# davidbau/rewriting

Hardware: NVIDIA H100
Metric: StyleGAN2-256 images/sec (higher is better)
Workload: dtype bf16x3 (3-term split bf16 operands, fp32 accumulate; fp32 in/out)

## Files before the change

rewriting_b200/csrc/conv_tc.cu:

```cuda
#include <cstdlib>
#include <cstring>

#include "rw_common.cuh"
#include "rw_kernels.h"

namespace rw {

namespace {

constexpr int BM = 128;
constexpr int BN = 128;
constexpr int BK = 64;
constexpr int MMA_K = 16;
constexpr int kStages = 3;
constexpr int kNumThreads = 288;
constexpr int kTmaWarp = 8;
constexpr int kChunkKB = 8;

struct ConvSmem {
  static constexpr int kABytes = BM * BK * 2;
  static constexpr int kBBytes = BN * BK * 2;
  static constexpr int kStageBytes = 2 * kABytes + 2 * kBBytes;
  static constexpr int kTotal = kStages * kStageBytes + 1024  + 256 ;
};

struct Barriers {
  uint64_t full[kStages];
  uint64_t empty[kStages];
};

__device__ __forceinline__ void decode_tile(int tile, int nphase, int nsched, int& ph, int& mn) {
  mn = tile / nphase;
  ph = tile - mn * nphase;
  if (nphase > 1) ph = (ph + ((nsched % nphase) == 0 ? tile / nsched : mn)) % nphase;
}

template <int EPI>
__global__ void __launch_bounds__(kNumThreads, 1)
conv_tc_kernel(const __grid_constant__ CUtensorMap map_a_hi,
               const __grid_constant__ CUtensorMap map_a_lo,
               const __grid_constant__ CUtensorMap map_w_hi,
               const __grid_constant__ CUtensorMap map_w_lo, const ConvTcParams p) {
  extern __shared__ uint8_t smem_raw[];
  uint8_t* smem = reinterpret_cast<uint8_t*>((reinterpret_cast<uintptr_t>(smem_raw) + 1023) &
                                             ~static_cast<uintptr_t>(1023));
  using S = ConvSmem;
  Barriers* bars = reinterpret_cast<Barriers*>(smem + kStages * S::kStageBytes);

  const int warp = threadIdx.x >> 5;
  const int lane = threadIdx.x & 31;
  const int nsched = gridDim.x;

  const int m_tiles = (p.rows + BM - 1) / BM;
  const int n_tiles = p.Cout / BN;
  const int mn_tiles = m_tiles * n_tiles;
  const int num_tiles = mn_tiles * p.nphase;
  const int kb_per_tap = p.Cin / BK;

  if (warp == kTmaWarp && lane == 0) {
    tma_prefetch_desc(&map_a_hi);
    tma_prefetch_desc(&map_a_lo);
    tma_prefetch_desc(&map_w_hi);
    tma_prefetch_desc(&map_w_lo);
    for (int s = 0; s < kStages; ++s) {
      mbar_init(&bars->full[s], 1);
      mbar_init(&bars->empty[s], 2);
    }
    fence_mbar_init();
  }
  __syncthreads();

  if (warp == kTmaWarp) {
    if (lane == 0) {
      int stage = 0;
      uint32_t phase = 0;
      for (int tile = blockIdx.x; tile < num_tiles; tile += nsched) {
        int ph, mn;
        decode_tile(tile, p.nphase, nsched, ph, mn);
        const int n0 = (mn % n_tiles) * BN;
        const int m0 = (mn / n_tiles) * BM;
        for (int t = 0; t < p.ph_ntaps[ph]; ++t) {
          const int arow = m0 + p.ph_shift[ph][t];
          const int wcol = p.ph_kofs[ph][t];
          const int acol = p.ph_acol[ph][t];
          for (int kb = 0; kb < kb_per_tap; ++kb) {
            mbar_wait(&bars->empty[stage], phase ^ 1u);
            uint8_t* st = smem + stage * S::kStageBytes;
            mbar_expect_tx(&bars->full[stage], S::kStageBytes);
            tma_load_2d(st, &map_a_hi, &bars->full[stage], acol + kb * BK, arow);
            tma_load_2d(st + S::kABytes, &map_a_lo, &bars->full[stage], acol + kb * BK, arow);
            tma_load_2d(st + 2 * S::kABytes, &map_w_hi, &bars->full[stage], wcol + kb * BK, n0);
            tma_load_2d(st + 2 * S::kABytes + S::kBBytes, &map_w_lo, &bars->full[stage],
                        wcol + kb * BK, n0);
            if (++stage == kStages) { stage = 0; phase ^= 1u; }
          }
        }
      }
    }
    return;
  }

  const int wg = threadIdx.x >> 7;
  const int g = lane >> 2, c = lane & 3;
  const int img = p.Hp * p.Wp;
  int stage = 0;
  uint32_t phase = 0;
  for (int tile = blockIdx.x; tile < num_tiles; tile += nsched) {
    int ph, mn;
    decode_tile(tile, p.nphase, nsched, ph, mn);
    const int num_kb = p.ph_ntaps[ph] * kb_per_tap;
    const int n_tile = mn % n_tiles;
    const int n0 = n_tile * BN;
    const int m0 = (mn / n_tiles) * BM;

    float acc[64], d[64];
#pragma unroll
    for (int j = 0; j < 64; ++j) acc[j] = 0.f;
    for (int kb0 = 0; kb0 < num_kb; kb0 += kChunkKB) {
      const int kb_end = (kb0 + kChunkKB < num_kb) ? kb0 + kChunkKB : num_kb;
      for (int kb = kb0; kb < kb_end; ++kb) {
        mbar_wait(&bars->full[stage], phase);
        const uint32_t sa = smem_u32(smem + stage * S::kStageBytes);
        const uint64_t da_hi = make_smem_desc(sa + wg * (S::kABytes / 2), 16, 1024);
        const uint64_t da_lo = make_smem_desc(sa + S::kABytes + wg * (S::kABytes / 2), 16, 1024);
        const uint64_t db_hi = make_smem_desc(sa + 2 * S::kABytes, 16, 1024);
        const uint64_t db_lo = make_smem_desc(sa + 2 * S::kABytes + S::kBBytes, 16, 1024);
        wgmma_fence();
#pragma unroll
        for (int kk = 0; kk < BK / MMA_K; ++kk) {
          const uint64_t adv = static_cast<uint64_t>((kk * MMA_K * 2) >> 4);
          wgmma_m64n128<0, 0>(d, da_lo + adv, db_hi + adv, ((kb - kb0) | kk) != 0);
          wgmma_m64n128<0, 0>(d, da_hi + adv, db_lo + adv, 1u);
          wgmma_m64n128<0, 0>(d, da_hi + adv, db_hi + adv, 1u);
        }
        wgmma_commit();
        wgmma_wait<0>();
        if ((threadIdx.x & 127) == 0) mbar_arrive(&bars->empty[stage]);
        if (++stage == kStages) { stage = 0; phase ^= 1u; }
      }
#pragma unroll
      for (int j = 0; j < 64; ++j) acc[j] += d[j];
    }

#pragma unroll
    for (int i = 0; i < 2; ++i) {
      const int prow = m0 + wg * 64 + (warp & 3) * 16 + g + 8 * i;
      const int b = prow / img;
      const int rem = prow - b * img;
      const int yy = rem / p.Wp;
      const int xx = rem - yy * p.Wp;
      const int Hv = p.ph_Hv[ph], Wv = p.ph_Wv[ph];
      const bool in_rows = prow < p.rows;
      const bool valid = in_rows && (yy < Hv) && (xx < Wv);
      const float* scl = (p.scale_bo && in_rows) ? p.scale_bo + static_cast<size_t>(b) * p.Cout : nullptr;
      float* outp = (p.out != nullptr && p.out_mode == 0 && valid)
                        ? p.out + p.ph_out_ofs[ph] + static_cast<size_t>(b) * p.out_sb +
                              static_cast<size_t>(yy) * p.out_sy + static_cast<size_t>(xx) * p.out_sx
                        : nullptr;
      if (EPI == 1 || !valid) {
        if (scl && (EPI == 1 || p.out_mode == 1)) {
#pragma unroll
          for (int j = 0; j < 16; ++j) {
            const float2 sv = __ldg(reinterpret_cast<const float2*>(scl + n0 + 8 * j + 2 * c));
            acc[4 * j + 2 * i] *= sv.x;
            acc[4 * j + 2 * i + 1] *= sv.y;
          }
        }
        if (EPI == 1 && outp) {
#pragma unroll
          for (int j = 0; j < 16; ++j)
#pragma unroll
            for (int e = 0; e < 2; ++e)
              outp[static_cast<size_t>(n0 + 8 * j + 2 * c + e) * p.out_sc] = acc[4 * j + 2 * i + e];
        }
      } else {
        float nz = 0.f;
        if (p.noise != nullptr)
          nz = __ldg(p.noise_w) * __ldg(p.noise + static_cast<size_t>(b) * p.noise_bstride +
                                        static_cast<size_t>(yy) * Wv + xx);
        const float act_gain = p.act_gain != 0.f ? p.act_gain : 1.4142135623730951f;
#pragma unroll
        for (int j = 0; j < 16; ++j)
#pragma unroll
          for (int e = 0; e < 2; ++e) {
            const int o = n0 + 8 * j + 2 * c + e;
            float t = acc[4 * j + 2 * i + e];
            if (scl) t *= __ldg(scl + o);
            t += nz;
            if (p.bias) t += __ldg(p.bias + o);
            if (p.act) t = (t > 0.f ? t : 0.2f * t) * act_gain;
            acc[4 * j + 2 * i + e] = t;
            if (outp) outp[static_cast<size_t>(o) * p.out_sc] = t;
          }
      }
      if (EPI == 0 && p.rgb_w != nullptr) {
        const float* rw0 = p.rgb_w + (static_cast<size_t>(valid ? b : 0) * 3) * p.Cout;
#pragma unroll
        for (int half = 0; half < 2; ++half) {
          float r0 = 0.f, r1 = 0.f, r2 = 0.f;
          if (valid) {
#pragma unroll
            for (int j = 8 * half; j < 8 * half + 8; ++j)
#pragma unroll
              for (int e = 0; e < 2; ++e) {
                const int o = n0 + 8 * j + 2 * c + e;
                const float t = acc[4 * j + 2 * i + e];
                r0 = fmaf(__ldg(rw0 + o), t, r0);
                r1 = fmaf(__ldg(rw0 + p.Cout + o), t, r1);
                r2 = fmaf(__ldg(rw0 + 2 * p.Cout + o), t, r2);
              }
          }
#pragma unroll
          for (int s = 1; s < 4; s <<= 1) {
            r0 += __shfl_xor_sync(0xffffffffu, r0, s);
            r1 += __shfl_xor_sync(0xffffffffu, r1, s);
            r2 += __shfl_xor_sync(0xffffffffu, r2, s);
          }
          if (valid && c == 0) {
            const size_t hw = static_cast<size_t>(Hv) * Wv;
            float* rp = p.rgb_part + ((static_cast<size_t>(n_tile * 2 + half) * p.B + b) * 3) * hw +
                        static_cast<size_t>(yy) * Wv + xx;
            rp[0] = r0;
            rp[hw] = r1;
            rp[2 * hw] = r2;
          }
        }
      }
      if (p.out != nullptr && p.out_mode == 1 && in_rows) {
        float* orow = p.out + (static_cast<size_t>(ph) * p.rows + prow) * p.Cout + n0 + 2 * c;
#pragma unroll
        for (int j = 0; j < 16; ++j)
          *reinterpret_cast<float2*>(orow + 8 * j) = make_float2(acc[4 * j + 2 * i], acc[4 * j + 2 * i + 1]);
      }
      if (EPI == 0 && p.next_hi != nullptr && in_rows) {
        const float* ns = p.next_scale + static_cast<size_t>(valid ? b : 0) * p.Cout + n0 + 2 * c;
        const size_t ofs = static_cast<size_t>(prow) * p.Cout + n0 + 2 * c;
        uint32_t* nh = reinterpret_cast<uint32_t*>(static_cast<__nv_bfloat16*>(p.next_hi) + ofs);
        uint32_t* nl = reinterpret_cast<uint32_t*>(static_cast<__nv_bfloat16*>(p.next_lo) + ofs);
#pragma unroll
        for (int j = 0; j < 16; ++j) {
          float k0 = 0.f, k1 = 0.f;
          if (valid) {
            const float2 sv = __ldg(reinterpret_cast<const float2*>(ns + 8 * j));
            k0 = sv.x * acc[4 * j + 2 * i];
            k1 = sv.y * acc[4 * j + 2 * i + 1];
          }
          const __nv_bfloat162 hh = __floats2bfloat162_rn(k0, k1);
          const float2 hf = __bfloat1622float2(hh);
          const __nv_bfloat162 ll = __floats2bfloat162_rn(k0 - hf.x, k1 - hf.y);
          nh[4 * j] = *reinterpret_cast<const uint32_t*>(&hh);
          nl[4 * j] = *reinterpret_cast<const uint32_t*>(&ll);
        }
      }
    }
  }
}

}

template <int EPI>
static int conv_tc_launch_epi(const ConvTcParams& p, const void* a_hi, const void* a_lo,
                              const void* w_hi, const void* w_lo, int wk_total,
                              cudaStream_t stream) {
  CUtensorMap ma_hi, ma_lo, mw_hi, mw_lo;
  int rc;
  const int a_cols = p.a_cols > 0 ? p.a_cols : p.Cin;
  if ((rc = make_tmap_2d_bf16(&ma_hi, a_hi, a_cols, p.rows, (uint64_t)a_cols * 2, BK, BM))) return rc;
  if ((rc = make_tmap_2d_bf16(&ma_lo, a_lo, a_cols, p.rows, (uint64_t)a_cols * 2, BK, BM))) return rc;
  if ((rc = make_tmap_2d_bf16(&mw_hi, w_hi, wk_total, p.Cout, (uint64_t)wk_total * 2, BK, BN)))
    return rc;
  if ((rc = make_tmap_2d_bf16(&mw_lo, w_lo, wk_total, p.Cout, (uint64_t)wk_total * 2, BK, BN)))
    return rc;

  static bool attr_set = false;
  if (!attr_set) {
    rc = check_cuda(cudaFuncSetAttribute(conv_tc_kernel<EPI>,
                                         cudaFuncAttributeMaxDynamicSharedMemorySize, ConvSmem::kTotal),
                    "conv_tc smem attr");
    if (rc) return rc;
    attr_set = true;
  }
  const int m_tiles = (p.rows + BM - 1) / BM;
  const int n_tiles = p.Cout / BN;
  const int num_tiles = m_tiles * n_tiles * p.nphase;
  int sched = device_sm_count();
  if (sched > num_tiles) sched = num_tiles;
  conv_tc_kernel<EPI><<<sched, kNumThreads, ConvSmem::kTotal, stream>>>(ma_hi, ma_lo, mw_hi, mw_lo, p);
  return check_cuda(cudaGetLastError(), "conv_tc launch");
}

int conv_tc_launch(const ConvTcParams& p, const void* a_hi, const void* a_lo, const void* w_hi,
                   const void* w_lo, int wk_total, cudaStream_t stream) {
  if (p.Cin % BK != 0 || p.Cout % BN != 0 || p.nphase < 1 || p.nphase > 4 || p.rows <= 0) {
    set_last_error("conv_tc: unsupported shape Cin=%d Cout=%d nphase=%d rows=%d", p.Cin, p.Cout,
                   p.nphase, p.rows);
    return RW_ERR_BAD_ARG;
  }
  for (int i = 0; i < p.nphase; ++i)
    if (p.ph_ntaps[i] < 1 || p.ph_ntaps[i] > 9) {
      set_last_error("conv_tc: phase %d has %d taps", i, p.ph_ntaps[i]);
      return RW_ERR_BAD_ARG;
    }
  const bool lean = !p.noise && !p.bias && !p.act && !p.rgb_w && !p.rgb_part && !p.next_hi &&
                    p.out != nullptr && (reinterpret_cast<uintptr_t>(p.scale_bo) & 7u) == 0;
  if (lean) return conv_tc_launch_epi<1>(p, a_hi, a_lo, w_hi, w_lo, wk_total, stream);
  return conv_tc_launch_epi<0>(p, a_hi, a_lo, w_hi, w_lo, wk_total, stream);
}

}
```

rewriting_b200/csrc/rw_common.cuh:

```cuda
#pragma once
#include <cuda_runtime.h>
#include <cuda_bf16.h>
#include <cuda.h>
#include <stdint.h>

namespace rw {

enum : int {
  RW_OK = 0,
  RW_ERR_BAD_ARG = -1,
  RW_ERR_CUDA = -2,
  RW_ERR_NO_DRIVER_SYMBOL = -3,
  RW_ERR_UNSUPPORTED = -4,
};
void set_last_error(const char* fmt, ...);
int check_cuda(cudaError_t e, const char* what);

#ifndef RW_SPIN_LIMIT
#define RW_SPIN_LIMIT (1u << 26)
#endif

__device__ __forceinline__ uint32_t smem_u32(const void* p) {
  return static_cast<uint32_t>(__cvta_generic_to_shared(p));
}

__device__ __forceinline__ uint32_t lane_id() { return threadIdx.x & 31u; }

__device__ __forceinline__ bool elect_one() {
  uint32_t pred = 0;
  asm volatile(
      "{\n\t.reg .pred P;\n\t"
      "elect.sync _|P, 0xffffffff;\n\t"
      "selp.u32 %0, 1, 0, P;\n\t}\n"
      : "=r"(pred));
  return pred != 0;
}

__device__ __forceinline__ void mbar_init(uint64_t* bar, uint32_t count) {
  asm volatile("mbarrier.init.shared::cta.b64 [%0], %1;\n" ::"r"(smem_u32(bar)), "r"(count));
}
__device__ __forceinline__ void fence_mbar_init() {
  asm volatile("fence.mbarrier_init.release.cluster;\n" ::: "memory");
}
__device__ __forceinline__ void fence_proxy_async_smem() {
  asm volatile("fence.proxy.async.shared::cta;\n" ::: "memory");
}
__device__ __forceinline__ void mbar_expect_tx(uint64_t* bar, uint32_t bytes) {
  asm volatile("mbarrier.arrive.expect_tx.shared::cta.b64 _, [%0], %1;\n" ::"r"(smem_u32(bar)),
               "r"(bytes)
               : "memory");
}
__device__ __forceinline__ void mbar_arrive(uint64_t* bar) {
  asm volatile("mbarrier.arrive.shared::cta.b64 _, [%0];\n" ::"r"(smem_u32(bar)) : "memory");
}
__device__ __forceinline__ bool mbar_try_wait(uint64_t* bar, uint32_t parity) {
  uint32_t ok;
  asm volatile(
      "{\n\t.reg .pred P;\n\t"
      "mbarrier.try_wait.parity.shared::cta.b64 P, [%1], %2;\n\t"
      "selp.u32 %0, 1, 0, P;\n\t}\n"
      : "=r"(ok)
      : "r"(smem_u32(bar)), "r"(parity)
      : "memory");
  return ok != 0;
}
__device__ __forceinline__ void mbar_wait(uint64_t* bar, uint32_t parity) {
  uint32_t spins = 0;
  while (!mbar_try_wait(bar, parity)) {
    if (++spins > RW_SPIN_LIMIT) __trap();
  }
}
__device__ __forceinline__ void named_bar_sync(int id, int count) {
  asm volatile("bar.sync %0, %1;\n" ::"r"(id), "r"(count) : "memory");
}

template <uint32_t N>
__device__ __forceinline__ void setmaxnreg_dec() {
  asm volatile("setmaxnreg.dec.sync.aligned.u32 %0;\n" ::"n"(N));
}
template <uint32_t N>
__device__ __forceinline__ void setmaxnreg_inc() {
  asm volatile("setmaxnreg.inc.sync.aligned.u32 %0;\n" ::"n"(N));
}

__device__ __forceinline__ void tma_prefetch_desc(const CUtensorMap* m) {
  asm volatile("prefetch.tensormap [%0];\n" ::"l"(reinterpret_cast<uint64_t>(m)) : "memory");
}
__device__ __forceinline__ void tma_load_2d(void* smem_dst, const CUtensorMap* m, uint64_t* bar,
                                            int32_t c_inner, int32_t c_outer) {
  asm volatile(
      "cp.async.bulk.tensor.2d.shared::cluster.global.mbarrier::complete_tx::bytes"
      " [%0], [%1, {%3, %4}], [%2];\n" ::"r"(smem_u32(smem_dst)),
      "l"(reinterpret_cast<uint64_t>(m)), "r"(smem_u32(bar)), "r"(c_inner), "r"(c_outer)
      : "memory");
}

__device__ __forceinline__ void wgmma_fence() {
  asm volatile("wgmma.fence.sync.aligned;\n" ::: "memory");
}
__device__ __forceinline__ void wgmma_commit() {
  asm volatile("wgmma.commit_group.sync.aligned;\n" ::: "memory");
}
template <int N>
__device__ __forceinline__ void wgmma_wait() {
  asm volatile("wgmma.wait_group.sync.aligned %0;\n" ::"n"(N) : "memory");
}
template <int TA, int TB>
__device__ __forceinline__ void wgmma_m64n128(float (&d)[64], uint64_t desc_a, uint64_t desc_b,
                                               uint32_t accumulate) {
  asm volatile(
      "{\n\t.reg .pred p;\n\t"
      "setp.ne.b32 p, %66, 0;\n\t"
      "wgmma.mma_async.sync.aligned.m64n128k16.f32.bf16.bf16 "
      "{%0, %1, %2, %3, %4, %5, %6, %7, %8, %9, %10, %11, %12, %13, %14, %15, %16, %17, %18, %19, %20, %21, %22, %23, %24, %25, %26, %27, %28, %29, %30, %31, %32, %33, %34, %35, %36, %37, %38, %39, %40, %41, %42, %43, %44, %45, %46, %47, %48, %49, %50, %51, %52, %53, %54, %55, %56, %57, %58, %59, %60, %61, %62, %63}, "
      "%64, %65, p, 1, 1, %67, %68;\n\t}\n"
      : "+f"(d[0]), "+f"(d[1]), "+f"(d[2]), "+f"(d[3]), "+f"(d[4]), "+f"(d[5]), "+f"(d[6]), "+f"(d[7]),
        "+f"(d[8]), "+f"(d[9]), "+f"(d[10]), "+f"(d[11]), "+f"(d[12]), "+f"(d[13]), "+f"(d[14]), "+f"(d[15]),
        "+f"(d[16]), "+f"(d[17]), "+f"(d[18]), "+f"(d[19]), "+f"(d[20]), "+f"(d[21]), "+f"(d[22]), "+f"(d[23]),
        "+f"(d[24]), "+f"(d[25]), "+f"(d[26]), "+f"(d[27]), "+f"(d[28]), "+f"(d[29]), "+f"(d[30]), "+f"(d[31]),
        "+f"(d[32]), "+f"(d[33]), "+f"(d[34]), "+f"(d[35]), "+f"(d[36]), "+f"(d[37]), "+f"(d[38]), "+f"(d[39]),
        "+f"(d[40]), "+f"(d[41]), "+f"(d[42]), "+f"(d[43]), "+f"(d[44]), "+f"(d[45]), "+f"(d[46]), "+f"(d[47]),
        "+f"(d[48]), "+f"(d[49]), "+f"(d[50]), "+f"(d[51]), "+f"(d[52]), "+f"(d[53]), "+f"(d[54]), "+f"(d[55]),
        "+f"(d[56]), "+f"(d[57]), "+f"(d[58]), "+f"(d[59]), "+f"(d[60]), "+f"(d[61]), "+f"(d[62]), "+f"(d[63])
      : "l"(desc_a), "l"(desc_b), "r"(accumulate), "n"(TA), "n"(TB));
}
template <int TA, int TB>
__device__ __forceinline__ void wgmma_m64n144(float (&d)[72], uint64_t desc_a, uint64_t desc_b,
                                               uint32_t accumulate) {
  asm volatile(
      "{\n\t.reg .pred p;\n\t"
      "setp.ne.b32 p, %74, 0;\n\t"
      "wgmma.mma_async.sync.aligned.m64n144k16.f32.bf16.bf16 "
      "{%0, %1, %2, %3, %4, %5, %6, %7, %8, %9, %10, %11, %12, %13, %14, %15, %16, %17, %18, %19, %20, %21, %22, %23, %24, %25, %26, %27, %28, %29, %30, %31, %32, %33, %34, %35, %36, %37, %38, %39, %40, %41, %42, %43, %44, %45, %46, %47, %48, %49, %50, %51, %52, %53, %54, %55, %56, %57, %58, %59, %60, %61, %62, %63, %64, %65, %66, %67, %68, %69, %70, %71}, "
      "%72, %73, p, 1, 1, %75, %76;\n\t}\n"
      : "+f"(d[0]), "+f"(d[1]), "+f"(d[2]), "+f"(d[3]), "+f"(d[4]), "+f"(d[5]), "+f"(d[6]), "+f"(d[7]),
        "+f"(d[8]), "+f"(d[9]), "+f"(d[10]), "+f"(d[11]), "+f"(d[12]), "+f"(d[13]), "+f"(d[14]), "+f"(d[15]),
        "+f"(d[16]), "+f"(d[17]), "+f"(d[18]), "+f"(d[19]), "+f"(d[20]), "+f"(d[21]), "+f"(d[22]), "+f"(d[23]),
        "+f"(d[24]), "+f"(d[25]), "+f"(d[26]), "+f"(d[27]), "+f"(d[28]), "+f"(d[29]), "+f"(d[30]), "+f"(d[31]),
        "+f"(d[32]), "+f"(d[33]), "+f"(d[34]), "+f"(d[35]), "+f"(d[36]), "+f"(d[37]), "+f"(d[38]), "+f"(d[39]),
        "+f"(d[40]), "+f"(d[41]), "+f"(d[42]), "+f"(d[43]), "+f"(d[44]), "+f"(d[45]), "+f"(d[46]), "+f"(d[47]),
        "+f"(d[48]), "+f"(d[49]), "+f"(d[50]), "+f"(d[51]), "+f"(d[52]), "+f"(d[53]), "+f"(d[54]), "+f"(d[55]),
        "+f"(d[56]), "+f"(d[57]), "+f"(d[58]), "+f"(d[59]), "+f"(d[60]), "+f"(d[61]), "+f"(d[62]), "+f"(d[63]),
        "+f"(d[64]), "+f"(d[65]), "+f"(d[66]), "+f"(d[67]), "+f"(d[68]), "+f"(d[69]), "+f"(d[70]), "+f"(d[71])
      : "l"(desc_a), "l"(desc_b), "r"(accumulate), "n"(TA), "n"(TB));
}

__host__ __device__ __forceinline__ uint64_t make_smem_desc(uint32_t saddr, uint32_t lbo_bytes,
                                                            uint32_t sbo_bytes, uint32_t layout = 1) {
  uint64_t d = 0;
  d |= static_cast<uint64_t>((saddr >> 4) & 0x3FFFu);
  d |= static_cast<uint64_t>((lbo_bytes >> 4) & 0x3FFFu) << 16;
  d |= static_cast<uint64_t>((sbo_bytes >> 4) & 0x3FFFu) << 32;
  d |= static_cast<uint64_t>(layout) << 62;
  return d;
}

__device__ __forceinline__ void split_bf16(float x, __nv_bfloat16& hi, __nv_bfloat16& lo) {
  hi = __float2bfloat16_rn(x);
  lo = __float2bfloat16_rn(x - __bfloat162float(hi));
}

int make_tmap_2d_bf16(CUtensorMap* out, const void* base, uint64_t inner, uint64_t outer,
                      uint64_t row_stride_bytes, uint32_t box_inner, uint32_t box_outer);

int device_sm_count();

}
```

Baseline: 1476.

## Use 2-CTA clusters with multicast weight TMA, deeper pipeline, warp-specialized registers

Pairs CTAs into clusters of two that share the weight tile, each loading half of B and multicasting it to both CTAs, with the empty barriers released across the cluster. BK drops to 32 with a 64B swizzle so that 7 pipeline stages fit in shared memory. Consumers now keep one wgmma group in flight (wait<1>) and release the previous stage. Thread count rises to 384 with setmaxnreg splitting registers between producer and consumer warps. The aim is to cut weight load traffic and hide latency, at the cost of cluster synchronization and scheduling constraints.

Result: faster. 1535, median of 6 (+4.0%).

```diff
diff --git a/rewriting_b200/csrc/conv_tc.cu b/rewriting_b200/csrc/conv_tc.cu
--- a/rewriting_b200/csrc/conv_tc.cu
+++ b/rewriting_b200/csrc/conv_tc.cu
@@ -10,19 +10,23 @@
 
 constexpr int BM = 128;
 constexpr int BN = 128;
-constexpr int BK = 64;
+constexpr int BK = 32;
 constexpr int MMA_K = 16;
-constexpr int kStages = 3;
-constexpr int kNumThreads = 288;
+constexpr int kStages = 7;
+constexpr int kNumThreads = 384;
 constexpr int kTmaWarp = 8;
-constexpr int kChunkKB = 8;
+constexpr uint32_t kProducerRegs = 40;
+constexpr uint32_t kConsumerRegs = 232;
+constexpr int kCluster = 2;
+constexpr int kChunkKB = 16;
 
 struct ConvSmem {
   static constexpr int kABytes = BM * BK * 2;
   static constexpr int kBBytes = BN * BK * 2;
   static constexpr int kStageBytes = 2 * kABytes + 2 * kBBytes;
-  static constexpr int kTotal = kStages * kStageBytes + 1024  + 256 ;
+  static constexpr int kTotal = kStages * kStageBytes + 512  + 256 ;
 };
+static_assert(ConvSmem::kTotal <= 232448, "conv_tc: shared memory over the per-block limit");
 
 struct Barriers {
   uint64_t full[kStages];
@@ -42,19 +46,21 @@
                const __grid_constant__ CUtensorMap map_w_hi,
                const __grid_constant__ CUtensorMap map_w_lo, const ConvTcParams p) {
   extern __shared__ uint8_t smem_raw[];
-  uint8_t* smem = reinterpret_cast<uint8_t*>((reinterpret_cast<uintptr_t>(smem_raw) + 1023) &
-                                             ~static_cast<uintptr_t>(1023));
+  uint8_t* smem = reinterpret_cast<uint8_t*>((reinterpret_cast<uintptr_t>(smem_raw) + 511) &
+                                             ~static_cast<uintptr_t>(511));
   using S = ConvSmem;
   Barriers* bars = reinterpret_cast<Barriers*>(smem + kStages * S::kStageBytes);
 
-  const int warp = threadIdx.x >> 5;
+  const int warp = __shfl_sync(0xffffffffu, static_cast<int>(threadIdx.x >> 5), 0);
   const int lane = threadIdx.x & 31;
-  const int nsched = gridDim.x;
+  const int rank = static_cast<int>(cluster_ctarank());
+  const int nsched = static_cast<int>(num_clusters_x());
+  const int first_unit = static_cast<int>(cluster_id_x());
 
   const int m_tiles = (p.rows + BM - 1) / BM;
   const int n_tiles = p.Cout / BN;
-  const int mn_tiles = m_tiles * n_tiles;
-  const int num_tiles = mn_tiles * p.nphase;
+  const int mn_units = (m_tiles + kCluster - 1) / kCluster * n_tiles;
+  const int num_units = mn_units * p.nphase;
   const int kb_per_tap = p.Cin / BK;
 
   if (warp == kTmaWarp && lane == 0) {
@@ -64,21 +70,194 @@
     tma_prefetch_desc(&map_w_lo);
     for (int s = 0; s < kStages; ++s) {
       mbar_init(&bars->full[s], 1);
-      mbar_init(&bars->empty[s], 2);
+      mbar_init(&bars->empty[s], 2 * kCluster);
     }
     fence_mbar_init();
   }
-  __syncthreads();
-
-  if (warp == kTmaWarp) {
-    if (lane == 0) {
+  cluster_sync();
+
+  if (warp < kTmaWarp) {
+    setmaxnreg_inc<kConsumerRegs>();
+    const int wg = threadIdx.x >> 7;
+    const int c = lane & 3;
+    const int img = p.Hp * p.Wp;
+    auto release = [&](int s) {
+      if ((threadIdx.x & 127) == 0) {
+#pragma unroll
+        for (int r = 0; r < kCluster; ++r) mbar_arrive_cluster(mapa_shared(&bars->empty[s], r));
+      }
+    };
+    int stage = 0;
+    uint32_t phase = 0;
+    for (int unit = first_unit; unit < num_units; unit += nsched) {
+      int ph, mn;
+      decode_tile(unit, p.nphase, nsched, ph, mn);
+      const int num_kb = p.ph_ntaps[ph] * kb_per_tap;
+      const int n_tile = mn % n_tiles;
+      const int n0 = n_tile * BN;
+      const int m0 = ((mn / n_tiles) * kCluster + rank) * BM;
+
+      float acc[64], d[64];
+#pragma unroll
+      for (int j = 0; j < 64; ++j) acc[j] = 0.f;
+      for (int kb0 = 0; kb0 < num_kb; kb0 += kChunkKB) {
+        const int kb_end = (kb0 + kChunkKB < num_kb) ? kb0 + kChunkKB : num_kb;
+        int held = -1;
+        for (int kb = kb0; kb < kb_end; ++kb) {
+          mbar_wait(&bars->full[stage], phase);
+          const uint32_t sa = smem_u32(smem + stage * S::kStageBytes);
+          const uint64_t da_hi = make_smem_desc(sa + wg * (S::kABytes / 2), 16, 512, 2);
+          const uint64_t da_lo = make_smem_desc(sa + S::kABytes + wg * (S::kABytes / 2), 16, 512, 2);
+          const uint64_t db_hi = make_smem_desc(sa + 2 * S::kABytes, 16, 512, 2);
+          const uint64_t db_lo = make_smem_desc(sa + 2 * S::kABytes + S::kBBytes, 16, 512, 2);
+          wgmma_fence();
+#pragma unroll
+          for (int kk = 0; kk < BK / MMA_K; ++kk) {
+            const uint64_t adv = static_cast<uint64_t>((kk * MMA_K * 2) >> 4);
+            wgmma_m64n128<0, 0>(d, da_lo + adv, db_hi + adv, ((kb - kb0) | kk) != 0);
+            wgmma_m64n128<0, 0>(d, da_hi + adv, db_lo + adv, 1u);
+            wgmma_m64n128<0, 0>(d, da_hi + adv, db_hi + adv, 1u);
+          }
+          wgmma_commit();
+          wgmma_wait<1>();
+          if (held >= 0) release(held);
+          held = stage;
+          if (++stage == kStages) { stage = 0; phase ^= 1u; }
+        }
+        wgmma_wait<0>();
+        release(held);
+#pragma unroll
+        for (int j = 0; j < 64; ++j) acc[j] += d[j];
+      }
+
+      uint32_t tid;
+      asm volatile("mov.u32 %0, %%tid.x;\n" : "=r"(tid));
+      const int row0 = m0 + ((tid >> 7) << 6) + (((tid >> 5) & 3) << 4) + ((tid & 31) >> 2);
+#pragma unroll
+      for (int i = 0; i < 2; ++i) {
+        const int prow = row0 + 8 * i;
+        const int b = prow / img;
+        const int rem = prow - b * img;
+        const int yy = rem / p.Wp;
+        const int xx = rem - yy * p.Wp;
+        const int Hv = p.ph_Hv[ph], Wv = p.ph_Wv[ph];
+        const bool in_rows = prow < p.rows;
+        const bool valid = in_rows && (yy < Hv) && (xx < Wv);
+        const float* scl = (p.scale_bo && in_rows) ? p.scale_bo + static_cast<size_t>(b) * p.Cout : nullptr;
+        float* outp = (p.out != nullptr && p.out_mode == 0 && valid)
+                          ? p.out + p.ph_out_ofs[ph] + static_cast<size_t>(b) * p.out_sb +
+                                static_cast<size_t>(yy) * p.out_sy + static_cast<size_t>(xx) * p.out_sx
+                          : nullptr;
+        if (EPI == 1 || !valid) {
+          if (scl && (EPI == 1 || p.out_mode == 1)) {
+#pragma unroll
+            for (int j = 0; j < 16; ++j) {
+              const float2 sv = __ldg(reinterpret_cast<const float2*>(scl + n0 + 8 * j + 2 * c));
+              acc[4 * j + 2 * i] *= sv.x;
+              acc[4 * j + 2 * i + 1] *= sv.y;
+            }
+          }
+          if (EPI == 1 && outp) {
+#pragma unroll
+            for (int j = 0; j < 16; ++j)
+#pragma unroll
+              for (int e = 0; e < 2; ++e)
+                outp[static_cast<size_t>(n0 + 8 * j + 2 * c + e) * p.out_sc] = acc[4 * j + 2 * i + e];
+          }
+        } else {
+          float nz = 0.f;
+          if (p.noise != nullptr)
+            nz = __ldg(p.noise_w) * __ldg(p.noise + static_cast<size_t>(b) * p.noise_bstride +
+                                          static_cast<size_t>(yy) * Wv + xx);
+          const float act_gain = p.act_gain != 0.f ? p.act_gain : 1.4142135623730951f;
+#pragma unroll
+          for (int j = 0; j < 16; ++j)
+#pragma unroll
+            for (int e = 0; e < 2; ++e) {
+              const int o = n0 + 8 * j + 2 * c + e;
+              float t = acc[4 * j + 2 * i + e];
+              if (scl) t *= __ldg(scl + o);
+              t += nz;
+              if (p.bias) t += __ldg(p.bias + o);
+              if (p.act) t = (t > 0.f ? t : 0.2f * t) * act_gain;
+              acc[4 * j + 2 * i + e] = t;
+              if (outp) outp[static_cast<size_t>(o) * p.out_sc] = t;
+            }
+        }
+        if (EPI == 0 && p.rgb_w != nullptr) {
+          const float* rw0 = p.rgb_w + (static_cast<size_t>(valid ? b : 0) * 3) * p.Cout;
+#pragma unroll
+          for (int half = 0; half < 2; ++half) {
+            float r0 = 0.f, r1 = 0.f, r2 = 0.f;
+            if (valid) {
+#pragma unroll
+              for (int j = 8 * half; j < 8 * half + 8; ++j)
+#pragma unroll
+                for (int e = 0; e < 2; ++e) {
+                  const int o = n0 + 8 * j + 2 * c + e;
+                  const float t = acc[4 * j + 2 * i + e];
+                  r0 = fmaf(__ldg(rw0 + o), t, r0);
+                  r1 = fmaf(__ldg(rw0 + p.Cout + o), t, r1);
+                  r2 = fmaf(__ldg(rw0 + 2 * p.Cout + o), t, r2);
+                }
+            }
+#pragma unroll
+            for (int s = 1; s < 4; s <<= 1) {
+              r0 += __shfl_xor_sync(0xffffffffu, r0, s);
+              r1 += __shfl_xor_sync(0xffffffffu, r1, s);
+              r2 += __shfl_xor_sync(0xffffffffu, r2, s);
+            }
+            if (valid && c == 0) {
+              const size_t hw = static_cast<size_t>(Hv) * Wv;
+              float* rp = p.rgb_part + ((static_cast<size_t>(n_tile * 2 + half) * p.B + b) * 3) * hw +
+                          static_cast<size_t>(yy) * Wv + xx;
+              rp[0] = r0;
+              rp[hw] = r1;
+              rp[2 * hw] = r2;
+            }
+          }
+        }
+        if (p.out != nullptr && p.out_mode == 1 && in_rows) {
+          float* orow = p.out + (static_cast<size_t>(ph) * p.rows + prow) * p.Cout + n0 + 2 * c;
+#pragma unroll
+          for (int j = 0; j < 16; ++j)
+            *reinterpret_cast<float2*>(orow + 8 * j) = make_float2(acc[4 * j + 2 * i], acc[4 * j + 2 * i + 1]);
+        }
+        if (EPI == 0 && p.next_hi != nullptr && in_rows) {
+          const float* ns = p.next_scale + static_cast<size_t>(valid ? b : 0) * p.Cout + n0 + 2 * c;
+          const size_t ofs = static_cast<size_t>(prow) * p.Cout + n0 + 2 * c;
+          uint32_t* nh = reinterpret_cast<uint32_t*>(static_cast<__nv_bfloat16*>(p.next_hi) + ofs);
+          uint32_t* nl = reinterpret_cast<uint32_t*>(static_cast<__nv_bfloat16*>(p.next_lo) + ofs);
+#pragma unroll
+          for (int j = 0; j < 16; ++j) {
+            float k0 = 0.f, k1 = 0.f;
+            if (valid) {
+              const float2 sv = __ldg(reinterpret_cast<const float2*>(ns + 8 * j));
+              k0 = sv.x * acc[4 * j + 2 * i];
+              k1 = sv.y * acc[4 * j + 2 * i + 1];
+            }
+            const __nv_bfloat162 hh = __floats2bfloat162_rn(k0, k1);
+            const float2 hf = __bfloat1622float2(hh);
+            const __nv_bfloat162 ll = __floats2bfloat162_rn(k0 - hf.x, k1 - hf.y);
+            nh[4 * j] = *reinterpret_cast<const uint32_t*>(&hh);
+            nl[4 * j] = *reinterpret_cast<const uint32_t*>(&ll);
+          }
+        }
+      }
+    }
+  } else {
+    setmaxnreg_dec<kProducerRegs>();
+    if (warp == kTmaWarp && lane == 0) {
+      constexpr uint16_t kMask = (1u << kCluster) - 1;
+      constexpr int kBSlice = BN / kCluster;
+      const uint32_t b_off = 2 * S::kABytes + rank * (S::kBBytes / kCluster);
       int stage = 0;
       uint32_t phase = 0;
-      for (int tile = blockIdx.x; tile < num_tiles; tile += nsched) {
+      for (int unit = first_unit; unit < num_units; unit += nsched) {
         int ph, mn;
-        decode_tile(tile, p.nphase, nsched, ph, mn);
-        const int n0 = (mn % n_tiles) * BN;
-        const int m0 = (mn / n_tiles) * BM;
+        decode_tile(unit, p.nphase, nsched, ph, mn);
+        const int n0 = (mn % n_tiles) * BN + rank * kBSlice;
+        const int m0 = ((mn / n_tiles) * kCluster + rank) * BM;
         for (int t = 0; t < p.ph_ntaps[ph]; ++t) {
           const int arow = m0 + p.ph_shift[ph][t];
           const int wcol = p.ph_kofs[ph][t];
@@ -89,171 +268,18 @@
             mbar_expect_tx(&bars->full[stage], S::kStageBytes);
             tma_load_2d(st, &map_a_hi, &bars->full[stage], acol + kb * BK, arow);
             tma_load_2d(st + S::kABytes, &map_a_lo, &bars->full[stage], acol + kb * BK, arow);
-            tma_load_2d(st + 2 * S::kABytes, &map_w_hi, &bars->full[stage], wcol + kb * BK, n0);
-            tma_load_2d(st + 2 * S::kABytes + S::kBBytes, &map_w_lo, &bars->full[stage],
-                        wcol + kb * BK, n0);
+            tma_load_2d_multicast(st + b_off, &map_w_hi, &bars->full[stage], wcol + kb * BK, n0,
+                                  kMask);
+            tma_load_2d_multicast(st + b_off + S::kBBytes, &map_w_lo, &bars->full[stage],
+                                  wcol + kb * BK, n0, kMask);
             if (++stage == kStages) { stage = 0; phase ^= 1u; }
           }
         }
       }
     }
-    return;
+    __syncwarp();
   }
-
-  const int wg = threadIdx.x >> 7;
-  const int g = lane >> 2, c = lane & 3;
-  const int img = p.Hp * p.Wp;
-  int stage = 0;
-  uint32_t phase = 0;
-  for (int tile = blockIdx.x; tile < num_tiles; tile += nsched) {
-    int ph, mn;
-    decode_tile(tile, p.nphase, nsched, ph, mn);
-    const int num_kb = p.ph_ntaps[ph] * kb_per_tap;
-    const int n_tile = mn % n_tiles;
-    const int n0 = n_tile * BN;
-    const int m0 = (mn / n_tiles) * BM;
-
-    float acc[64], d[64];
-#pragma unroll
-    for (int j = 0; j < 64; ++j) acc[j] = 0.f;
-    for (int kb0 = 0; kb0 < num_kb; kb0 += kChunkKB) {
-      const int kb_end = (kb0 + kChunkKB < num_kb) ? kb0 + kChunkKB : num_kb;
-      for (int kb = kb0; kb < kb_end; ++kb) {
-        mbar_wait(&bars->full[stage], phase);
-        const uint32_t sa = smem_u32(smem + stage * S::kStageBytes);
-        const uint64_t da_hi = make_smem_desc(sa + wg * (S::kABytes / 2), 16, 1024);
-        const uint64_t da_lo = make_smem_desc(sa + S::kABytes + wg * (S::kABytes / 2), 16, 1024);
-        const uint64_t db_hi = make_smem_desc(sa + 2 * S::kABytes, 16, 1024);
-        const uint64_t db_lo = make_smem_desc(sa + 2 * S::kABytes + S::kBBytes, 16, 1024);
-        wgmma_fence();
-#pragma unroll
-        for (int kk = 0; kk < BK / MMA_K; ++kk) {
-          const uint64_t adv = static_cast<uint64_t>((kk * MMA_K * 2) >> 4);
-          wgmma_m64n128<0, 0>(d, da_lo + adv, db_hi + adv, ((kb - kb0) | kk) != 0);
-          wgmma_m64n128<0, 0>(d, da_hi + adv, db_lo + adv, 1u);
-          wgmma_m64n128<0, 0>(d, da_hi + adv, db_hi + adv, 1u);
-        }
-        wgmma_commit();
-        wgmma_wait<0>();
-        if ((threadIdx.x & 127) == 0) mbar_arrive(&bars->empty[stage]);
-        if (++stage == kStages) { stage = 0; phase ^= 1u; }
-      }
-#pragma unroll
-      for (int j = 0; j < 64; ++j) acc[j] += d[j];
-    }
-
-#pragma unroll
-    for (int i = 0; i < 2; ++i) {
-      const int prow = m0 + wg * 64 + (warp & 3) * 16 + g + 8 * i;
-      const int b = prow / img;
-      const int rem = prow - b * img;
-      const int yy = rem / p.Wp;
-      const int xx = rem - yy * p.Wp;
-      const int Hv = p.ph_Hv[ph], Wv = p.ph_Wv[ph];
-      const bool in_rows = prow < p.rows;
-      const bool valid = in_rows && (yy < Hv) && (xx < Wv);
-      const float* scl = (p.scale_bo && in_rows) ? p.scale_bo + static_cast<size_t>(b) * p.Cout : nullptr;
-      float* outp = (p.out != nullptr && p.out_mode == 0 && valid)
-                        ? p.out + p.ph_out_ofs[ph] + static_cast<size_t>(b) * p.out_sb +
-                              static_cast<size_t>(yy) * p.out_sy + static_cast<size_t>(xx) * p.out_sx
-                        : nullptr;
-      if (EPI == 1 || !valid) {
-        if (scl && (EPI == 1 || p.out_mode == 1)) {
-#pragma unroll
-          for (int j = 0; j < 16; ++j) {
-            const float2 sv = __ldg(reinterpret_cast<const float2*>(scl + n0 + 8 * j + 2 * c));
-            acc[4 * j + 2 * i] *= sv.x;
-            acc[4 * j + 2 * i + 1] *= sv.y;
-          }
-        }
-        if (EPI == 1 && outp) {
-#pragma unroll
-          for (int j = 0; j < 16; ++j)
-#pragma unroll
-            for (int e = 0; e < 2; ++e)
-              outp[static_cast<size_t>(n0 + 8 * j + 2 * c + e) * p.out_sc] = acc[4 * j + 2 * i + e];
-        }
-      } else {
-        float nz = 0.f;
-        if (p.noise != nullptr)
-          nz = __ldg(p.noise_w) * __ldg(p.noise + static_cast<size_t>(b) * p.noise_bstride +
-                                        static_cast<size_t>(yy) * Wv + xx);
-        const float act_gain = p.act_gain != 0.f ? p.act_gain : 1.4142135623730951f;
-#pragma unroll
-        for (int j = 0; j < 16; ++j)
-#pragma unroll
-          for (int e = 0; e < 2; ++e) {
-            const int o = n0 + 8 * j + 2 * c + e;
-            float t = acc[4 * j + 2 * i + e];
-            if (scl) t *= __ldg(scl + o);
-            t += nz;
-            if (p.bias) t += __ldg(p.bias + o);
-            if (p.act) t = (t > 0.f ? t : 0.2f * t) * act_gain;
-            acc[4 * j + 2 * i + e] = t;
-            if (outp) outp[static_cast<size_t>(o) * p.out_sc] = t;
-          }
-      }
-      if (EPI == 0 && p.rgb_w != nullptr) {
-        const float* rw0 = p.rgb_w + (static_cast<size_t>(valid ? b : 0) * 3) * p.Cout;
-#pragma unroll
-        for (int half = 0; half < 2; ++half) {
-          float r0 = 0.f, r1 = 0.f, r2 = 0.f;
-          if (valid) {
-#pragma unroll
-            for (int j = 8 * half; j < 8 * half + 8; ++j)
-#pragma unroll
-              for (int e = 0; e < 2; ++e) {
-                const int o = n0 + 8 * j + 2 * c + e;
-                const float t = acc[4 * j + 2 * i + e];
-                r0 = fmaf(__ldg(rw0 + o), t, r0);
-                r1 = fmaf(__ldg(rw0 + p.Cout + o), t, r1);
-                r2 = fmaf(__ldg(rw0 + 2 * p.Cout + o), t, r2);
-              }
-          }
-#pragma unroll
-          for (int s = 1; s < 4; s <<= 1) {
-            r0 += __shfl_xor_sync(0xffffffffu, r0, s);
-            r1 += __shfl_xor_sync(0xffffffffu, r1, s);
-            r2 += __shfl_xor_sync(0xffffffffu, r2, s);
-          }
-          if (valid && c == 0) {
-            const size_t hw = static_cast<size_t>(Hv) * Wv;
-            float* rp = p.rgb_part + ((static_cast<size_t>(n_tile * 2 + half) * p.B + b) * 3) * hw +
-                        static_cast<size_t>(yy) * Wv + xx;
-            rp[0] = r0;
-            rp[hw] = r1;
-            rp[2 * hw] = r2;
-          }
-        }
-      }
-      if (p.out != nullptr && p.out_mode == 1 && in_rows) {
-        float* orow = p.out + (static_cast<size_t>(ph) * p.rows + prow) * p.Cout + n0 + 2 * c;
-#pragma unroll
-        for (int j = 0; j < 16; ++j)
-          *reinterpret_cast<float2*>(orow + 8 * j) = make_float2(acc[4 * j + 2 * i], acc[4 * j + 2 * i + 1]);
-      }
-      if (EPI == 0 && p.next_hi != nullptr && in_rows) {
-        const float* ns = p.next_scale + static_cast<size_t>(valid ? b : 0) * p.Cout + n0 + 2 * c;
-        const size_t ofs = static_cast<size_t>(prow) * p.Cout + n0 + 2 * c;
-        uint32_t* nh = reinterpret_cast<uint32_t*>(static_cast<__nv_bfloat16*>(p.next_hi) + ofs);
-        uint32_t* nl = reinterpret_cast<uint32_t*>(static_cast<__nv_bfloat16*>(p.next_lo) + ofs);
-#pragma unroll
-        for (int j = 0; j < 16; ++j) {
-          float k0 = 0.f, k1 = 0.f;
-          if (valid) {
-            const float2 sv = __ldg(reinterpret_cast<const float2*>(ns + 8 * j));
-            k0 = sv.x * acc[4 * j + 2 * i];
-            k1 = sv.y * acc[4 * j + 2 * i + 1];
-          }
-          const __nv_bfloat162 hh = __floats2bfloat162_rn(k0, k1);
-          const float2 hf = __bfloat1622float2(hh);
-          const __nv_bfloat162 ll = __floats2bfloat162_rn(k0 - hf.x, k1 - hf.y);
-          nh[4 * j] = *reinterpret_cast<const uint32_t*>(&hh);
-          nl[4 * j] = *reinterpret_cast<const uint32_t*>(&ll);
-        }
-      }
-    }
-  }
+  cluster_sync();
 }
 
 }
@@ -264,34 +290,56 @@
                               cudaStream_t stream) {
   CUtensorMap ma_hi, ma_lo, mw_hi, mw_lo;
   int rc;
-  const int a_cols = p.a_cols > 0 ? p.a_cols : p.Cin;
-  if ((rc = make_tmap_2d_bf16(&ma_hi, a_hi, a_cols, p.rows, (uint64_t)a_cols * 2, BK, BM))) return rc;
-  if ((rc = make_tmap_2d_bf16(&ma_lo, a_lo, a_cols, p.rows, (uint64_t)a_cols * 2, BK, BM))) return rc;
-  if ((rc = make_tmap_2d_bf16(&mw_hi, w_hi, wk_total, p.Cout, (uint64_t)wk_total * 2, BK, BN)))
-    return rc;
-  if ((rc = make_tmap_2d_bf16(&mw_lo, w_lo, wk_total, p.Cout, (uint64_t)wk_total * 2, BK, BN)))
-    return rc;
-
-  static bool attr_set = false;
-  if (!attr_set) {
+  const uint64_t a_cols = p.a_cols > 0 ? p.a_cols : p.Cin;
+  const uint64_t a_dims[2] = {a_cols, static_cast<uint64_t>(p.rows)}, a_str[1] = {a_cols * 2};
+  const uint64_t w_dims[2] = {static_cast<uint64_t>(wk_total), static_cast<uint64_t>(p.Cout)};
+  const uint64_t w_str[1] = {static_cast<uint64_t>(wk_total) * 2};
+  const uint32_t a_box[2] = {BK, BM}, w_box[2] = {BK, BN / kCluster};
+  if ((rc = make_tmap_nd_bf16(&ma_hi, a_hi, 2, a_dims, a_str, a_box, nullptr, 3))) return rc;
+  if ((rc = make_tmap_nd_bf16(&ma_lo, a_lo, 2, a_dims, a_str, a_box, nullptr, 3))) return rc;
+  if ((rc = make_tmap_nd_bf16(&mw_hi, w_hi, 2, w_dims, w_str, w_box, nullptr, 3))) return rc;
+  if ((rc = make_tmap_nd_bf16(&mw_lo, w_lo, 2, w_dims, w_str, w_box, nullptr, 3))) return rc;
+
+  cudaLaunchConfig_t cfg = {};
+  cudaLaunchAttribute attr[1];
+  attr[0].id = cudaLaunchAttributeClusterDimension;
+  attr[0].val.clusterDim.x = kCluster;
+  attr[0].val.clusterDim.y = 1;
+  attr[0].val.clusterDim.z = 1;
+  cfg.blockDim = dim3(kNumThreads);
+  cfg.dynamicSmemBytes = ConvSmem::kTotal;
+  cfg.stream = stream;
+  cfg.attrs = attr;
+  cfg.numAttrs = 1;
+  static int max_clusters = 0;
+  if (max_clusters == 0) {
     rc = check_cuda(cudaFuncSetAttribute(conv_tc_kernel<EPI>,
                                          cudaFuncAttributeMaxDynamicSharedMemorySize, ConvSmem::kTotal),
                     "conv_tc smem attr");
     if (rc) return rc;
-    attr_set = true;
+    cfg.gridDim = dim3(kCluster * (device_sm_count() / kCluster));
+    rc = check_cuda(cudaOccupancyMaxActiveClusters(&max_clusters, conv_tc_kernel<EPI>, &cfg),
+                    "conv_tc cluster occupancy");
+    if (rc) return rc;
+    if (max_clusters < 1) {
+      set_last_error("conv_tc: no cluster of %d CTAs fits on the device", kCluster);
+      return RW_ERR_UNSUPPORTED;
+    }
   }
   const int m_tiles = (p.rows + BM - 1) / BM;
   const int n_tiles = p.Cout / BN;
-  const int num_tiles = m_tiles * n_tiles * p.nphase;
-  int sched = device_sm_count();
-  if (sched > num_tiles) sched = num_tiles;
-  conv_tc_kernel<EPI><<<sched, kNumThreads, ConvSmem::kTotal, stream>>>(ma_hi, ma_lo, mw_hi, mw_lo, p);
+  const int num_units = (m_tiles + kCluster - 1) / kCluster * n_tiles * p.nphase;
+  const int clusters = max_clusters < num_units ? max_clusters : num_units;
+  cfg.gridDim = dim3(kCluster * clusters);
+  rc = check_cuda(cudaLaunchKernelEx(&cfg, conv_tc_kernel<EPI>, ma_hi, ma_lo, mw_hi, mw_lo, p),
+                  "conv_tc launch");
+  if (rc) return rc;
   return check_cuda(cudaGetLastError(), "conv_tc launch");
 }
 
 int conv_tc_launch(const ConvTcParams& p, const void* a_hi, const void* a_lo, const void* w_hi,
                    const void* w_lo, int wk_total, cudaStream_t stream) {
-  if (p.Cin % BK != 0 || p.Cout % BN != 0 || p.nphase < 1 || p.nphase > 4 || p.rows <= 0) {
+  if (p.Cin % 64 != 0 || p.Cout % BN != 0 || p.nphase < 1 || p.nphase > 4 || p.rows <= 0) {
     set_last_error("conv_tc: unsupported shape Cin=%d Cout=%d nphase=%d rows=%d", p.Cin, p.Cout,
                    p.nphase, p.rows);
     return RW_ERR_BAD_ARG;
diff --git a/rewriting_b200/csrc/rw_common.cuh b/rewriting_b200/csrc/rw_common.cuh
--- a/rewriting_b200/csrc/rw_common.cuh
+++ b/rewriting_b200/csrc/rw_common.cuh
@@ -74,6 +74,33 @@
   asm volatile("bar.sync %0, %1;\n" ::"r"(id), "r"(count) : "memory");
 }
 
+__device__ __forceinline__ uint32_t cluster_ctarank() {
+  uint32_t r;
+  asm volatile("mov.u32 %0, %%cluster_ctarank;\n" : "=r"(r));
+  return r;
+}
+__device__ __forceinline__ uint32_t cluster_id_x() {
+  uint32_t r;
+  asm volatile("mov.u32 %0, %%clusterid.x;\n" : "=r"(r));
+  return r;
+}
+__device__ __forceinline__ uint32_t num_clusters_x() {
+  uint32_t r;
+  asm volatile("mov.u32 %0, %%nclusterid.x;\n" : "=r"(r));
+  return r;
+}
+__device__ __forceinline__ void cluster_sync() {
+  asm volatile("barrier.cluster.arrive.release;\nbarrier.cluster.wait.acquire;\n" ::: "memory");
+}
+__device__ __forceinline__ uint32_t mapa_shared(const void* p, uint32_t rank) {
+  uint32_t r;
+  asm volatile("mapa.shared::cluster.u32 %0, %1, %2;\n" : "=r"(r) : "r"(smem_u32(p)), "r"(rank));
+  return r;
+}
+__device__ __forceinline__ void mbar_arrive_cluster(uint32_t cluster_addr) {
+  asm volatile("mbarrier.arrive.shared::cluster.b64 _, [%0];\n" ::"r"(cluster_addr) : "memory");
+}
+
 template <uint32_t N>
 __device__ __forceinline__ void setmaxnreg_dec() {
   asm volatile("setmaxnreg.dec.sync.aligned.u32 %0;\n" ::"n"(N));
@@ -92,6 +119,16 @@
       "cp.async.bulk.tensor.2d.shared::cluster.global.mbarrier::complete_tx::bytes"
       " [%0], [%1, {%3, %4}], [%2];\n" ::"r"(smem_u32(smem_dst)),
       "l"(reinterpret_cast<uint64_t>(m)), "r"(smem_u32(bar)), "r"(c_inner), "r"(c_outer)
+      : "memory");
+}
+__device__ __forceinline__ void tma_load_2d_multicast(void* smem_dst, const CUtensorMap* m,
+                                                      uint64_t* bar, int32_t c_inner,
+                                                      int32_t c_outer, uint16_t cta_mask) {
+  asm volatile(
+      "cp.async.bulk.tensor.2d.shared::cluster.global.mbarrier::complete_tx::bytes.multicast::cluster"
+      " [%0], [%1, {%3, %4}], [%2], %5;\n" ::"r"(smem_u32(smem_dst)),
+      "l"(reinterpret_cast<uint64_t>(m)), "r"(smem_u32(bar)), "r"(c_inner), "r"(c_outer),
+      "h"(cta_mask)
       : "memory");
 }
 
@@ -162,6 +199,9 @@
 
 int make_tmap_2d_bf16(CUtensorMap* out, const void* base, uint64_t inner, uint64_t outer,
                       uint64_t row_stride_bytes, uint32_t box_inner, uint32_t box_outer);
+int make_tmap_nd_bf16(CUtensorMap* out, const void* base, int rank, const uint64_t* dims,
+                      const uint64_t* strides_bytes, const uint32_t* box, const uint32_t* estrides,
+                      int swizzle);
 
 int device_sm_count();
 
```
